# IDEA-Research/MP-Former

Measured on AMD Instinct MI355X. Metric: training images/sec COCO-instance R50 1024x1024, higher is better.
Workload: dtype bf16 (backbone, decoder) + f32 (pixel decoder, losses), as the reference's AMP; 1 GPU; COCO-instance R50, 100 queries, 80 classes, 1024x1024: full train step = R50 backbone + MSDeformAttn pixel decoder (6 layers) + MP masked decoder (9 layers, NUM_DN 1) + Hungarian matching + 60 losses + backward + grad all-reduce + clip + AdamW; head_only_workload=False, global_batch=2, per_gpu_batch=2, parallelism=dp1, msda_offsets=init, full=False, autograd_threads=backward on the launch thread, miopen_find_db=shipped

## Files before the change

### mp_former_amd/csrc/gemm3_nt2.h

```cpp
constexpr int kN2T = 512;
constexpr int kN2Kc = 256 * 16;
constexpr int kN2Op = 2 * 4 * kN2Kc;
constexpr int kN2Stage = 2 * kN2Op;
constexpr int kN2Lds = 2 * kN2Stage;

struct AccN2 {
    f32x16 v[4][2];
    __device__ __forceinline__ void zero()
    {
#pragma unroll
        for (int i = 0; i < 4; ++i)
#pragma unroll
            for (int j = 0; j < 2; ++j)
#pragma unroll
                for (int e = 0; e < 16; ++e) v[i][j][e] = 0.f;
    }
    __device__ __forceinline__ void step(const unsigned char* st, int a_base, int b_base, int lane)
    {
        const int r32 = lane & 31, gh = lane >> 5;
#pragma unroll
        for (int kh = 0; kh < 2; ++kh) {
            const int kc = 2 * kh + gh;
            const int sw = (r32 ^ (2 * kc)) * 16;
            f16x8 fb[2][2];
#pragma unroll
            for (int pl = 0; pl < 2; ++pl)
#pragma unroll
                for (int t = 0; t < 2; ++t) fb[pl][t] = as_fragh(*reinterpret_cast<const uint4*>(st + kN2Op + b_base + (pl * 4 + kc) * kN2Kc + t * 512 + sw));
#pragma unroll
            for (int i = 0; i < 4; ++i) {
                const f16x8 fah = as_fragh(*reinterpret_cast<const uint4*>(st + a_base + (0 * 4 + kc) * kN2Kc + i * 512 + sw));
                const f16x8 fal = as_fragh(*reinterpret_cast<const uint4*>(st + a_base + (1 * 4 + kc) * kN2Kc + i * 512 + sw));
#pragma unroll
                for (int j = 0; j < 2; ++j) v[i][j] = __builtin_amdgcn_mfma_f32_32x32x16_f16(fb[1][j], fah, v[i][j], 0, 0, 0);
#pragma unroll
                for (int j = 0; j < 2; ++j) v[i][j] = __builtin_amdgcn_mfma_f32_32x32x16_f16(fb[0][j], fal, v[i][j], 0, 0, 0);
#pragma unroll
                for (int j = 0; j < 2; ++j) v[i][j] = __builtin_amdgcn_mfma_f32_32x32x16_f16(fb[0][j], fah, v[i][j], 0, 0, 0);
            }
        }
    }
};

template <bool CV>
__device__ __forceinline__ void gemm3_nt2_tile(const G3N& p, const int tile, unsigned char* lds)
{
    float sc_a, sc_b, inv_a, inv_b;
    h2_scale(amax_read(p.a_amax), &sc_a, &inv_a);
    h2_scale(amax_read(p.b_amax), &sc_b, &inv_b);
    const int tn = tile % p.tiles_n, tm = (tile / p.tiles_n) % p.tiles_m, sp = tile / (p.tiles_n * p.tiles_m);
    const int m0 = tm * 256, n0 = tn * 256;
    const int r_begin = sp * p.rows_per_split, r_end = min(p.R, r_begin + p.rows_per_split);
    const int tid = threadIdx.x, lane = tid & 63, wave = tid >> 6;
    const int wr = wave >> 2, wc = wave & 3;

    const int col = tid & 255, kc0 = __builtin_amdgcn_readfirstlane(tid >> 8);
    const __amdgpu_buffer_rsrc_t ars = __builtin_amdgcn_make_buffer_rsrc(const_cast<float*>(p.a), 0, p.a_bytes, 0x00020000);
    const __amdgpu_buffer_rsrc_t brs = __builtin_amdgcn_make_buffer_rsrc(const_cast<float*>(p.b), 0, p.b_bytes, 0x00020000);
    const int acolb = (m0 + col) * 4, bcolb = (CV ? (n0 % p.cv_cin) + col : n0 + col) * 4;
    const int ldab = (int)p.lda * 4, ldbb = (int)p.ldb * 4;
    int cv_dy = 0, cv_dx = 0, cv_sh = 0, cvx0 = 0, cvy0 = 0, cvx1 = 0, cvy1 = 0;
    if constexpr (CV) {
        const int tap = n0 / p.cv_cin;
        cv_dy = tap / 3 - 1; cv_dx = tap % 3 - 1;
        cv_sh = cv_dy * p.cv_W + cv_dx;
        const int rb0 = r_begin + kc0 * 8, rb1 = rb0 + 16;
        cvx0 = rb0 % p.cv_W; cvy0 = (rb0 / p.cv_W) % p.cv_H;
        cvx1 = rb1 % p.cv_W; cvy1 = (rb1 / p.cv_W) % p.cv_H;
    }
    (void)cv_dy; (void)cv_dx; (void)cv_sh;
    float xa0[8], xa1[8], xb0[8], xb1[8];
    float csa = 0.f;
    const bool want_csa = p.csum_a && tn == 0;

#define N2_LOAD_A(r0, TAIL)                                                                                      \
    {                                                                                                            \
        _Pragma("unroll") for (int j = 0; j < 8; ++j) {                                                          \
            const int q0 = (r0) + kc0 * 8 + j, q1 = q0 + 16;                                                     \
            const int c0 = TAIL ? min(q0, r_end - 1) : q0, c1 = TAIL ? min(q1, r_end - 1) : q1;                  \
            float va0 = __int_as_float(__builtin_amdgcn_raw_buffer_load_b32(ars, acolb, c0 * ldab, 0));          \
            float va1 = __int_as_float(__builtin_amdgcn_raw_buffer_load_b32(ars, acolb, c1 * ldab, 0));          \
            if (TAIL) { va0 = q0 < r_end ? va0 : 0.f; va1 = q1 < r_end ? va1 : 0.f; }                            \
            xa0[j] = va0; xa1[j] = va1;                                                                          \
        }                                                                                                        \
    }
#define N2_LOAD_B(r0, TAIL)                                                                                      \
    {                                                                                                            \
        _Pragma("unroll") for (int j = 0; j < 8; ++j) {                                                          \
            const int q0 = (r0) + kc0 * 8 + j, q1 = q0 + 16;                                                     \
            int c0 = TAIL ? min(q0, r_end - 1) : q0, c1 = TAIL ? min(q1, r_end - 1) : q1;                        \
            if constexpr (CV) { c0 = min(max(c0 + cv_sh, 0), p.R - 1); c1 = min(max(c1 + cv_sh, 0), p.R - 1); }  \
            float vb0 = __int_as_float(__builtin_amdgcn_raw_buffer_load_b32(brs, bcolb, c0 * ldbb, 0));          \
            float vb1 = __int_as_float(__builtin_amdgcn_raw_buffer_load_b32(brs, bcolb, c1 * ldbb, 0));          \
            if constexpr (CV) {                                                                                  \
                const bool ok0 = (unsigned)(cvy0 + cv_dy) < (unsigned)p.cv_H && (unsigned)(cvx0 + j + cv_dx) < (unsigned)p.cv_W; \
                const bool ok1 = (unsigned)(cvy1 + cv_dy) < (unsigned)p.cv_H && (unsigned)(cvx1 + j + cv_dx) < (unsigned)p.cv_W; \
                vb0 = ok0 ? vb0 : 0.f; vb1 = ok1 ? vb1 : 0.f;                                                    \
            }                                                                                                    \
            if (TAIL) { vb0 = q0 < r_end ? vb0 : 0.f; vb1 = q1 < r_end ? vb1 : 0.f; }                            \
            xb0[j] = vb0; xb1[j] = vb1;                                                                          \
        }                                                                                                        \
        if constexpr (CV) {                                              \
            cvx0 += kBK; while (cvx0 >= p.cv_W) { cvx0 -= p.cv_W; cvy0 = cvy0 + 1 == p.cv_H ? 0 : cvy0 + 1; }    \
            cvx1 += kBK; while (cvx1 >= p.cv_W) { cvx1 -= p.cv_W; cvy1 = cvy1 + 1 == p.cv_H ? 0 : cvy1 + 1; }    \
        }                                                                                                        \
    }
#define N2_LOAD(r0, TAIL) { N2_LOAD_A(r0, TAIL) N2_LOAD_B(r0, TAIL) }

    AccN2 acc;
    acc.zero();
    const int a_base = wr * 128 * 16, b_base = wc * 64 * 16;
    const int sl0 = (col ^ (2 * kc0)) * 16, sl1 = (col ^ (2 * kc0 + 4)) * 16;

    if (r_begin + kBK <= r_end) N2_LOAD(r_begin, false) else N2_LOAD(r_begin, true);
    int s = 0;
    for (int r0 = r_begin; r0 < r_end; r0 += kBK, s ^= 1) {
        unsigned char* st = lds + s * kN2Stage;
        uint4 h, l;
        const bool full_next = r0 + 2 * kBK <= r_end, some_next = r0 + kBK < r_end;
        split8h(make_float4(xa0[0], xa0[1], xa0[2], xa0[3]), make_float4(xa0[4], xa0[5], xa0[6], xa0[7]), sc_a, &h, &l);
        *reinterpret_cast<uint4*>(st + (0 * 4 + kc0) * kN2Kc + sl0) = h;
        *reinterpret_cast<uint4*>(st + (1 * 4 + kc0) * kN2Kc + sl0) = l;
        split8h(make_float4(xa1[0], xa1[1], xa1[2], xa1[3]), make_float4(xa1[4], xa1[5], xa1[6], xa1[7]), sc_a, &h, &l);
        *reinterpret_cast<uint4*>(st + (0 * 4 + kc0 + 2) * kN2Kc + sl1) = h;
        *reinterpret_cast<uint4*>(st + (1 * 4 + kc0 + 2) * kN2Kc + sl1) = l;
        if (want_csa) {
#pragma unroll
            for (int j = 0; j < 8; ++j) csa += xa0[j] + xa1[j];
        }
        if (full_next) N2_LOAD_A(r0 + kBK, false) else if (some_next) N2_LOAD_A(r0 + kBK, true);
        split8h(make_float4(xb0[0], xb0[1], xb0[2], xb0[3]), make_float4(xb0[4], xb0[5], xb0[6], xb0[7]), sc_b, &h, &l);
        *reinterpret_cast<uint4*>(st + kN2Op + (0 * 4 + kc0) * kN2Kc + sl0) = h;
        *reinterpret_cast<uint4*>(st + kN2Op + (1 * 4 + kc0) * kN2Kc + sl0) = l;
        split8h(make_float4(xb1[0], xb1[1], xb1[2], xb1[3]), make_float4(xb1[4], xb1[5], xb1[6], xb1[7]), sc_b, &h, &l);
        *reinterpret_cast<uint4*>(st + kN2Op + (0 * 4 + kc0 + 2) * kN2Kc + sl1) = h;
        *reinterpret_cast<uint4*>(st + kN2Op + (1 * 4 + kc0 + 2) * kN2Kc + sl1) = l;
        if (full_next) N2_LOAD_B(r0 + kBK, false) else if (some_next) N2_LOAD_B(r0 + kBK, true);
        ws_barrier();
        acc.step(st, a_base, b_base, lane);
    }
#undef N2_LOAD
#undef N2_LOAD_A
#undef N2_LOAD_B

    float* cp = p.c + (int64_t)sp * p.c_ss;
    {
        const int r32 = lane & 31, gh = lane >> 5;
#pragma unroll
        for (int j = 0; j < 2; ++j)
#pragma unroll
            for (int i = 0; i < 4; ++i)
#pragma unroll
                for (int q = 0; q < 4; ++q) {
                    const int m = m0 + wr * 128 + i * 32 + r32, n = n0 + wc * 64 + j * 32 + 8 * q + 4 * gh;
                    float4 o = make_float4(acc.v[i][j][4 * q], acc.v[i][j][4 * q + 1], acc.v[i][j][4 * q + 2], acc.v[i][j][4 * q + 3]);
                    o = make_float4(o.x * inv_a * inv_b, o.y * inv_a * inv_b, o.z * inv_a * inv_b, o.w * inv_a * inv_b);
                    *reinterpret_cast<float4*>(cp + (int64_t)m * p.Ndim + n) = o;
                }
    }
    if (want_csa) {
        __syncthreads();
        float* red = reinterpret_cast<float*>(lds);
        if (tid < 256) red[tid] = csa;
        __syncthreads();
        if (tid >= 256) red[col] += csa;
        __syncthreads();
        if (tid < 256) p.csum_a[(int64_t)sp * p.csa_ss + m0 + tid] = red[tid];
    }
}

__global__ __launch_bounds__(kN2T, 2) void gemm3_nt2_group_kernel(G3NG g)
{
    extern __shared__ __attribute__((aligned(16))) unsigned char n2_lds[];
    const int per_xcd = (g.ntiles + 7) >> 3;
    const int tile = ((int)blockIdx.x & 7) * per_xcd + ((int)blockIdx.x >> 3);
    if (tile >= g.ntiles) return;
    int i = 0;
    while (i + 1 < g.n_items && tile >= g.tile_end[i]) ++i;
    const int first = i ? g.tile_end[i - 1] : 0;
    gemm3_nt2_tile<false>(g.it[i], tile - first, n2_lds);
}

__global__ __launch_bounds__(kN2T, 2) void gemm3_nt2_conv_kernel(G3N p)
{
    extern __shared__ __attribute__((aligned(16))) unsigned char n2_lds[];
    const int per_xcd = (p.ntiles + 7) >> 3;
    const int tile = ((int)blockIdx.x & 7) * per_xcd + ((int)blockIdx.x >> 3);
    if (tile >= p.ntiles) return;
    gemm3_nt2_tile<true>(p, tile, n2_lds);
}
```

Baseline: 86.20 images/sec.

## Interleave next-stage LDS stores and global loads with MFMA in split-f16 GEMM

Restructures the main loop of the 3-pass split-f16 NT GEMM so the conversion and LDS stores for the next stage, plus the global loads for the stage after, are interleaved between the per-row-tile MFMA groups of the current stage. This replaces the previous load-then-compute order with one barrier per step. The aim is to hide conversion and memory latency behind matrix-core work. It adds a steady-state loop for full steps and a fallback loop for the tail, which raises code complexity and register pressure and may lower occupancy.

```diff
diff --git a/mp_former_amd/csrc/gemm3_nt2.h b/mp_former_amd/csrc/gemm3_nt2.h
--- a/mp_former_amd/csrc/gemm3_nt2.h
+++ b/mp_former_amd/csrc/gemm3_nt2.h
@@ -15,29 +15,36 @@
 #pragma unroll
                 for (int e = 0; e < 16; ++e) v[i][j][e] = 0.f;
     }
+    __device__ __forceinline__ void load_b(const unsigned char* st, int b_base, int lane, int kh, f16x8 (&fb)[2][2])
+    {
+        const int r32 = lane & 31, kc = 2 * kh + (lane >> 5);
+        const int sw = (r32 ^ (2 * kc)) * 16;
+#pragma unroll
+        for (int pl = 0; pl < 2; ++pl)
+#pragma unroll
+            for (int t = 0; t < 2; ++t) fb[pl][t] = as_fragh(*reinterpret_cast<const uint4*>(st + kN2Op + b_base + (pl * 4 + kc) * kN2Kc + t * 512 + sw));
+    }
+    __device__ __forceinline__ void tile_i(const unsigned char* st, int a_base, int lane, int kh, int i, const f16x8 (&fb)[2][2])
+    {
+        const int r32 = lane & 31, kc = 2 * kh + (lane >> 5);
+        const int sw = (r32 ^ (2 * kc)) * 16;
+        const f16x8 fah = as_fragh(*reinterpret_cast<const uint4*>(st + a_base + (0 * 4 + kc) * kN2Kc + i * 512 + sw));
+        const f16x8 fal = as_fragh(*reinterpret_cast<const uint4*>(st + a_base + (1 * 4 + kc) * kN2Kc + i * 512 + sw));
+#pragma unroll
+        for (int j = 0; j < 2; ++j) v[i][j] = __builtin_amdgcn_mfma_f32_32x32x16_f16(fb[1][j], fah, v[i][j], 0, 0, 0);
+#pragma unroll
+        for (int j = 0; j < 2; ++j) v[i][j] = __builtin_amdgcn_mfma_f32_32x32x16_f16(fb[0][j], fal, v[i][j], 0, 0, 0);
+#pragma unroll
+        for (int j = 0; j < 2; ++j) v[i][j] = __builtin_amdgcn_mfma_f32_32x32x16_f16(fb[0][j], fah, v[i][j], 0, 0, 0);
+    }
     __device__ __forceinline__ void step(const unsigned char* st, int a_base, int b_base, int lane)
     {
-        const int r32 = lane & 31, gh = lane >> 5;
 #pragma unroll
         for (int kh = 0; kh < 2; ++kh) {
-            const int kc = 2 * kh + gh;
-            const int sw = (r32 ^ (2 * kc)) * 16;
             f16x8 fb[2][2];
-#pragma unroll
-            for (int pl = 0; pl < 2; ++pl)
-#pragma unroll
-                for (int t = 0; t < 2; ++t) fb[pl][t] = as_fragh(*reinterpret_cast<const uint4*>(st + kN2Op + b_base + (pl * 4 + kc) * kN2Kc + t * 512 + sw));
-#pragma unroll
-            for (int i = 0; i < 4; ++i) {
-                const f16x8 fah = as_fragh(*reinterpret_cast<const uint4*>(st + a_base + (0 * 4 + kc) * kN2Kc + i * 512 + sw));
-                const f16x8 fal = as_fragh(*reinterpret_cast<const uint4*>(st + a_base + (1 * 4 + kc) * kN2Kc + i * 512 + sw));
-#pragma unroll
-                for (int j = 0; j < 2; ++j) v[i][j] = __builtin_amdgcn_mfma_f32_32x32x16_f16(fb[1][j], fah, v[i][j], 0, 0, 0);
-#pragma unroll
-                for (int j = 0; j < 2; ++j) v[i][j] = __builtin_amdgcn_mfma_f32_32x32x16_f16(fb[0][j], fal, v[i][j], 0, 0, 0);
-#pragma unroll
-                for (int j = 0; j < 2; ++j) v[i][j] = __builtin_amdgcn_mfma_f32_32x32x16_f16(fb[0][j], fah, v[i][j], 0, 0, 0);
-            }
+            load_b(st, b_base, lane, kh, fb);
+#pragma unroll
+            for (int i = 0; i < 4; ++i) tile_i(st, a_base, lane, kh, i, fb);
         }
     }
 };
@@ -113,32 +120,68 @@
     const int sl0 = (col ^ (2 * kc0)) * 16, sl1 = (col ^ (2 * kc0 + 4)) * 16;
 
     if (r_begin + kBK <= r_end) N2_LOAD(r_begin, false) else N2_LOAD(r_begin, true);
-    int s = 0;
-    for (int r0 = r_begin; r0 < r_end; r0 += kBK, s ^= 1) {
-        unsigned char* st = lds + s * kN2Stage;
-        uint4 h, l;
-        const bool full_next = r0 + 2 * kBK <= r_end, some_next = r0 + kBK < r_end;
-        split8h(make_float4(xa0[0], xa0[1], xa0[2], xa0[3]), make_float4(xa0[4], xa0[5], xa0[6], xa0[7]), sc_a, &h, &l);
-        *reinterpret_cast<uint4*>(st + (0 * 4 + kc0) * kN2Kc + sl0) = h;
-        *reinterpret_cast<uint4*>(st + (1 * 4 + kc0) * kN2Kc + sl0) = l;
-        split8h(make_float4(xa1[0], xa1[1], xa1[2], xa1[3]), make_float4(xa1[4], xa1[5], xa1[6], xa1[7]), sc_a, &h, &l);
-        *reinterpret_cast<uint4*>(st + (0 * 4 + kc0 + 2) * kN2Kc + sl1) = h;
-        *reinterpret_cast<uint4*>(st + (1 * 4 + kc0 + 2) * kN2Kc + sl1) = l;
-        if (want_csa) {
-#pragma unroll
-            for (int j = 0; j < 8; ++j) csa += xa0[j] + xa1[j];
-        }
-        if (full_next) N2_LOAD_A(r0 + kBK, false) else if (some_next) N2_LOAD_A(r0 + kBK, true);
-        split8h(make_float4(xb0[0], xb0[1], xb0[2], xb0[3]), make_float4(xb0[4], xb0[5], xb0[6], xb0[7]), sc_b, &h, &l);
-        *reinterpret_cast<uint4*>(st + kN2Op + (0 * 4 + kc0) * kN2Kc + sl0) = h;
-        *reinterpret_cast<uint4*>(st + kN2Op + (1 * 4 + kc0) * kN2Kc + sl0) = l;
-        split8h(make_float4(xb1[0], xb1[1], xb1[2], xb1[3]), make_float4(xb1[4], xb1[5], xb1[6], xb1[7]), sc_b, &h, &l);
-        *reinterpret_cast<uint4*>(st + kN2Op + (0 * 4 + kc0 + 2) * kN2Kc + sl1) = h;
-        *reinterpret_cast<uint4*>(st + kN2Op + (1 * 4 + kc0 + 2) * kN2Kc + sl1) = l;
-        if (full_next) N2_LOAD_B(r0 + kBK, false) else if (some_next) N2_LOAD_B(r0 + kBK, true);
+#define N2_PUT(x, sc, opnd, kc, sl)                                                                              \
+    {                                                                                                            \
+        uint4 h, l;                                                                                              \
+        split8h(make_float4(x[0], x[1], x[2], x[3]), make_float4(x[4], x[5], x[6], x[7]), sc, &h, &l);           \
+        *reinterpret_cast<uint4*>(sn + (opnd) + (0 * 4 + (kc)) * kN2Kc + (sl)) = h;                              \
+        *reinterpret_cast<uint4*>(sn + (opnd) + (1 * 4 + (kc)) * kN2Kc + (sl)) = l;                              \
+    }
+#define N2_CSA()                                                                                                 \
+    if (want_csa) {                                                                                              \
+        _Pragma("unroll") for (int j = 0; j < 8; ++j) csa += xa0[j] + xa1[j];                                    \
+    }
+#define N2_STAGE(k)                                                                                              \
+    {                                                                                                            \
+        unsigned char* sn = lds + ((k) & 1) * kN2Stage;                                                          \
+        const int rn = r_begin + ((k) + 1) * kBK;                                                                \
+        const bool full_next = rn + kBK <= r_end, some_next = rn < r_end;                         \
+        N2_PUT(xa0, sc_a, 0, kc0, sl0)                                                                           \
+        N2_PUT(xa1, sc_a, 0, kc0 + 2, sl1)                                                                       \
+        N2_CSA()                                                                                                 \
+        if (full_next) N2_LOAD_A(rn, false) else if (some_next) N2_LOAD_A(rn, true);                             \
+        N2_PUT(xb0, sc_b, kN2Op, kc0, sl0)                                                                       \
+        N2_PUT(xb1, sc_b, kN2Op, kc0 + 2, sl1)                                                                   \
+        if (full_next) N2_LOAD_B(rn, false) else if (some_next) N2_LOAD_B(rn, true);                             \
+    }
+    const int nsteps = (r_end - r_begin + kBK - 1) / kBK, nfull = (r_end - r_begin) / kBK;
+    N2_STAGE(0)
+    ws_barrier();
+    int k = 0;
+#pragma unroll 1
+    for (; k + 3 <= nfull; ++k) {
+        const unsigned char* st = lds + (k & 1) * kN2Stage;
+        unsigned char* sn = lds + ((k + 1) & 1) * kN2Stage;
+        const int rn = r_begin + (k + 2) * kBK;
+        f16x8 fb[2][2];
+        acc.load_b(st, b_base, lane, 0, fb);
+        acc.tile_i(st, a_base, lane, 0, 0, fb);
+        N2_PUT(xa0, sc_a, 0, kc0, sl0)
+        acc.tile_i(st, a_base, lane, 0, 1, fb);
+        N2_PUT(xa1, sc_a, 0, kc0 + 2, sl1)
+        N2_CSA()
+        acc.tile_i(st, a_base, lane, 0, 2, fb);
+        N2_LOAD_A(rn, false)
+        acc.tile_i(st, a_base, lane, 0, 3, fb);
+        acc.load_b(st, b_base, lane, 1, fb);
+        acc.tile_i(st, a_base, lane, 1, 0, fb);
+        N2_PUT(xb0, sc_b, kN2Op, kc0, sl0)
+        acc.tile_i(st, a_base, lane, 1, 1, fb);
+        N2_PUT(xb1, sc_b, kN2Op, kc0 + 2, sl1)
+        acc.tile_i(st, a_base, lane, 1, 2, fb);
+        N2_LOAD_B(rn, false)
+        acc.tile_i(st, a_base, lane, 1, 3, fb);
         ws_barrier();
-        acc.step(st, a_base, b_base, lane);
-    }
+    }
+#pragma unroll 1
+    for (; k < nsteps; ++k) {
+        acc.step(lds + (k & 1) * kN2Stage, a_base, b_base, lane);
+        if (k + 1 < nsteps) N2_STAGE(k + 1)
+        ws_barrier();
+    }
+#undef N2_STAGE
+#undef N2_CSA
+#undef N2_PUT
 #undef N2_LOAD
 #undef N2_LOAD_A
 #undef N2_LOAD_B
```

Result: no change. 87.00 images/sec (median of 6 runs) (+0.9%).
